# Immortalqx/pi-slam-fusion

Hardware: AMD Instinct MI355X
Metric: keyframes/sec fused (4000x3000 -> 256^2 tiles, 5-band) (higher is better)
Workload: dtype f32; 1 GPU; cfg-2/cfg-A: 4000x3000 BGR8 keyframes, serpentine sortie, Map2D.Scale=1, 5-band Laplacian, CV_32FC3 (ForceFloat=1) pyramids, frames resident in HBM; frames_per_rank=2646, sortie_frames_before_timing=20, lookahead=48, rendered_rank0=2666, culled_tiles_rank0=490117

## Files before the change

### include/pifusion.h

```cpp
#ifndef PIFUSION_H
#define PIFUSION_H
#include <stddef.h>
#include <stdint.h>

#ifdef __cplusplus
extern "C" {
#endif

#define PF_ELE_PIXELS 256

enum { PF_TYPE_NONE = 0, PF_TYPE_CPU = 1, PF_TYPE_GPU = 2, PF_TYPE_MULTIBAND = 3, PF_TYPE_RENDER = 4 };

enum { PF_8UC1 = 0, PF_8UC3 = 16, PF_8UC4 = 24, PF_16SC3 = 19, PF_32FC1 = 5, PF_32FC3 = 21 };

typedef struct pf_image {
    int         rows, cols, type;
    const void* data;
    size_t      step;
} pf_image;

typedef struct pf_options {
    int    band_number;
    int    force_float;
    int    high_quality_show;
// ... 126 lines not shown
int      pf_dist_blend_changed(pf_dist* d, int* xy, uint8_t* bgr, int cap);
int      pf_dist_save(pf_dist* d, const char* filename);
int      pf_dist_save_to_memory(pf_dist* d, uint8_t* bgr, int* rows, int* cols, int* tile_x0, int* tile_y0);
typedef struct pf_dist_stats {
    unsigned long long bytes_sent, bytes_received;
    unsigned long long strips_sent, strips_received, tiles, peers;
    double plan_ms, pack_ms, exchange_ms, compute_ms;
    unsigned long long verified;
} pf_dist_stats;
int      pf_dist_last_stats(pf_dist* d, pf_dist_stats* out);
typedef struct pf_strip_plan { int peer, ix, iy, dx, dy, tile; unsigned long long offset; } pf_strip_plan;
int      pf_dist_plan_blend(int nranks, int me, const int* counts, const int* lists3, const long long* caps, int high_quality,
                            const size_t halo_bytes9[9], pf_strip_plan* send, int send_cap, int* n_send,
                            pf_strip_plan* recv, int recv_cap, int* n_recv, int* mine_xy, int mine_cap, int* n_mine);
int      pf_dist_info(pf_dist* d, int* rank, int* nranks, const char** transport);
int      pf_dist_set_verify(pf_dist* d, int on);

int     pf_profile_enable(pf_map* m, int mode);
int     pf_profile_read(pf_map* m, int cap, const char** names, double* total_ms, long long* launches,
                        double* alg_bytes);
int     pf_profile_read_run(pf_map* m, int cap, const char** names, double* total_ms, long long* launches,
                            double* alg_bytes, double* alg_bytes_run);
int     pf_profile_reset(pf_map* m);
int     pf_render_stats(pf_map* m, double out4[4]);
int     pf_timer_read(pf_map* m, int cap, const char** names, long long* calls, double* mean_s, double* min_s, double* max_s);
int     pf_timer_reset(pf_map* m);
long long pf_debug_culled_tiles(pf_map* m);
long long pf_debug_culled_cells(pf_map* m);
double  pf_debug_level0_exact_px(pf_map* m);
int     pf_debug_render_log(pf_map* m, long long* out, int cap);
void    pf_set_cull(pf_map* m, int on);
void    pf_debug_form_counts(long long out[8]);
long long pf_debug_compact_launches(void);
int     pf_stats(pf_map* m, long long* rendered, long long* rejected, long long* dropped);
int     pf_reserve_tiles(pf_map* m, long long n_tiles);

#ifdef __cplusplus
}
#endif
#endif
```

### pi-slam-fusion_amd/__init__.py

```python
import ctypes as C
import os
import subprocess

import numpy as np

_HERE = os.path.dirname(os.path.abspath(__file__))
LIB_PATH = os.environ.get("PF_LIB") or os.path.join(_HERE, "libpifusion.so")
ELE_PIXELS = 256

NoType, TypeCPU, TypeGPU, TypeMultiBandCPU, TypeRender = 0, 1, 2, 3, 4
PF_8UC3, PF_8UC4, PF_16SC3, PF_32FC3 = 16, 24, 19, 21


def host_array(shape, dtype=np.uint8):
    n = int(np.prod(shape)) * np.dtype(dtype).itemsize
    p = lib().pf_host_alloc(n)
    if not p:
        raise MemoryError("pf_host_alloc(%d)" % n)
    buf = (C.c_uint8 * n).from_address(p)
    a = np.frombuffer(buf, dtype=dtype).reshape(shape)
    import weakref
    weakref.finalize(buf, lib().pf_host_free, p)
    return a

# ... 113 lines not shown
        L.pf_host_free.argtypes = [vp]; L.pf_host_free.restype = None
    if hasattr(L, "pf_blend_tiles_level") or not os.environ.get("PF_LIB"):
        L.pf_blend_tiles_level.argtypes = [vp, ip, C.c_int, C.c_int, vp, vp]
        L.pf_blend_changed_level.argtypes = [vp, C.c_int, ip, vp, C.c_int]
        L.pf_save_to_memory_level.argtypes = [vp, C.c_int, vp, ip, ip, ip, ip]
    L.pf_format_map_update.argtypes = [dp, dp, C.c_double, C.c_double, C.c_double, C.c_int, C.c_int, C.c_char_p, C.c_int]
    L.pf_map_update_command.argtypes = [vp, C.c_int, C.c_int, dp, C.c_char_p, C.c_int]
    L.pf_lnglat_from_distance.argtypes = [C.c_double, C.c_double, C.c_double, C.c_double, dp, dp]; L.pf_lnglat_from_distance.restype = None
    L.pf_normalize_using_weight_map.argtypes = [vp, vp, C.c_size_t]
    L.pf_mul_weight_map.argtypes = [vp, vp, C.c_size_t]
    L.pf_tile_owner.argtypes = [C.POINTER(Options), C.c_int, C.c_int]
    L.pf_halo_bytes.argtypes = [vp, C.c_int, C.c_int]; L.pf_halo_bytes.restype = C.c_size_t
    L.pf_halo_pack.argtypes = [vp, C.c_int, C.c_int, C.c_int, C.c_int, vp]
    L.pf_blend_tile_halo.argtypes = [vp, C.c_int, C.c_int, C.POINTER(vp), vp, vp]
    L.pf_tile_bytes.argtypes = [vp]; L.pf_tile_bytes.restype = C.c_size_t
    L.pf_tile_export.argtypes = [vp, C.c_int, C.c_int, vp]
    L.pf_tile_import.argtypes = [vp, C.c_int, C.c_int, vp]
    L.pf_dist_unique_id.argtypes = [vp]
    L.pf_dist_init_rccl.argtypes = [vp, vp, C.c_int, C.c_int]; L.pf_dist_init_rccl.restype = vp
    L.pf_dist_init_host.argtypes = [vp, C.c_int, C.c_int, EXCHANGE_FN, vp]; L.pf_dist_init_host.restype = vp
    L.pf_dist_destroy.argtypes = [vp]; L.pf_dist_destroy.restype = None
    L.pf_dist_blend_changed.argtypes = [vp, ip, vp, C.c_int]
    L.pf_dist_feed.argtypes = [vp, C.POINTER(Image), dp, C.c_int]
    L.pf_dist_feed_jpeg.argtypes = [vp, C.c_char_p, C.c_size_t, C.c_int, C.c_int, dp, C.c_int]
    L.pf_dist_save.argtypes = [vp, C.c_char_p]
    L.pf_dist_save_to_memory.argtypes = [vp, vp, ip, ip, ip, ip]
    L.pf_dist_last_stats.argtypes = [vp, C.POINTER(DistStats)]
    L.pf_dist_info.argtypes = [vp, ip, ip, C.POINTER(C.c_char_p)]
    L.pf_dist_set_verify.argtypes = [vp, C.c_int]
    L.pf_dist_plan_blend.argtypes = [C.c_int, C.c_int, ip, ip, C.POINTER(C.c_longlong), C.c_int, C.POINTER(C.c_size_t), vp, C.c_int, ip,
                                     vp, C.c_int, ip, ip, C.c_int, ip]
    if hasattr(L, "pf_debug_compact_launches") or not os.environ.get("PF_LIB"):
        L.pf_debug_compact_launches.argtypes = []; L.pf_debug_compact_launches.restype = C.c_longlong
    L.pf_profile_enable.argtypes = [vp, C.c_int]
    L.pf_profile_read.argtypes = [vp, C.c_int, C.POINTER(C.c_char_p), dp, C.POINTER(C.c_longlong), dp]
    if hasattr(L, "pf_profile_read_run") or not os.environ.get("PF_LIB"):
        L.pf_profile_read_run.argtypes = [vp, C.c_int, C.POINTER(C.c_char_p), dp, C.POINTER(C.c_longlong), dp, dp]
    L.pf_profile_reset.argtypes = [vp]
    L.pf_stats.argtypes = [vp, C.POINTER(C.c_longlong), C.POINTER(C.c_longlong), C.POINTER(C.c_longlong)]
    L.pf_reserve_tiles.argtypes = [vp, C.c_longlong]
    L.pf_debug_culled_tiles.argtypes = [vp]; L.pf_debug_culled_tiles.restype = C.c_longlong
    L.pf_set_cull.argtypes = [vp, C.c_int]; L.pf_set_cull.restype = None
    if hasattr(L, "pf_debug_render_log") or not os.environ.get("PF_LIB"):
        L.pf_debug_render_log.argtypes = [vp, C.POINTER(C.c_longlong), C.c_int]
    L.pf_debug_culled_cells.argtypes = [vp]; L.pf_debug_culled_cells.restype = C.c_longlong
    L.pf_debug_level0_exact_px.argtypes = [vp]; L.pf_debug_level0_exact_px.restype = C.c_double
    L.pf_render_stats.argtypes = [vp, dp]
    L.pf_timer_read.argtypes = [vp, C.c_int, C.POINTER(C.c_char_p), C.POINTER(C.c_longlong), dp, dp, dp]
    L.pf_timer_reset.argtypes = [vp]
    _lib = L
    return L


POSE7 = C.c_double * 7


def _pose(p):
    if isinstance(p, POSE7):
        return p, p
    a = np.ascontiguousarray(p, dtype=np.float64).reshape(-1)
    return a, a.ctypes.data_as(C.POINTER(C.c_double))


def default_options(**kw):
    o = Options()
    lib().pf_default_options(C.byref(o))
# ... 558 lines not shown
```

### pi-slam-fusion_amd/csrc/c_api.cpp

```cpp
#include "dist.hpp"
#include "jpeg_device.hpp"
#include "webtiles_plan.hpp"
#include <cerrno>
#include <map>
#include <string>
#include <sys/stat.h>
#include <cstdlib>
#include <cmath>
#include <cstdio>
#include <cstring>
#include <algorithm>
#include <vector>
#include <mutex>
#include <new>

using pf::FusionMap;

struct pf_map {
    FusionMap impl;
    pf::JpegDevice jpeg;
    pf_map(int t, bool th, const pf_options& o) : impl(t, th, o) {}
    ~pf_map() { if (impl.ok() && impl.use_device()) impl.sync(); }
};

// ... 27 lines not shown
    else if (!std::strcmp(key, "Map2D.Resolution")) o->resolution = v;
    else if (!std::strcmp(key, "Map2D.Scale")) o->scale = v;
    else if (!std::strcmp(key, "Device")) o->device = (int)v;
    else if (!std::strcmp(key, "Shard.Rank")) o->shard_rank = (int)v;
    else if (!std::strcmp(key, "Shard.Count")) o->shard_count = (int)v;
    else if (!std::strcmp(key, "Shard.Block")) o->shard_block = (int)v;
    else if (!std::strcmp(key, "Map2D.MaxQueue")) o->max_queue = (int)v;
    else if (!std::strcmp(key, "Fused")) o->fused = (int)v;
    else if (!std::strcmp(key, "Lookahead")) o->lookahead = (int)v;
    else return 0;
    return 1;
}

pf_map* pf_create(int type, int thread, const pf_options* opt)
{
    if (type == PF_TYPE_NONE || type == PF_TYPE_RENDER) return nullptr;
    pf_options o;
    if (opt) o = *opt; else pf_default_options(&o);
    pf_map* m = new (std::nothrow) pf_map(type, thread != 0, o);
    if (m && !m->impl.ok()) { delete m; return nullptr; }
    return m;
}

void pf_destroy(pf_map* m) { delete m; }
const char* pf_last_error(void) { return pf::last_error(); }

int pf_prepare(pf_map* m, const double plane[7], const double cam[6], int n, const pf_image* imgs, const double* poses7)
{ return m && m->impl.prepare(plane, cam, n, imgs, poses7); }

int pf_feed(pf_map* m, const pf_image* img, const double pose[7]) { return m && m->impl.feed(img, pose, false); }
int pf_feed_device(pf_map* m, const pf_image* img, const double pose[7]) { return m && m->impl.feed(img, pose, true); }
int pf_debug_phase_stamps(unsigned long long* out, int cap_blocks) { return pf::read_phase_stamps(out, cap_blocks); }
void pf_debug_form_counts(long long out[8]) { if (out) pf::read_form_counts(out); }
long long pf_debug_compact_launches(void) { return pf::read_compact_launches(); }
int pf_debug_render_log(pf_map* m, long long* out, int cap) { return m ? m->impl.render_log(out, cap) : 0; }
void pf_set_cull(pf_map* m, int on) { if (m) m->impl.set_cull(on != 0); }
long long pf_debug_culled_cells(pf_map* m) { return m ? m->impl.culled_cells() : 0; }
double pf_debug_level0_exact_px(pf_map* m) { return m ? m->impl.level0_exact_px() : 0; }
long long pf_debug_culled_tiles(pf_map* m) { return m ? m->impl.culled_tiles() : 0; }
int pf_debug_select_counts(unsigned long long* out, int reset) { return out ? pf::read_select_counts(out, reset) : 0; }
long pf_debug_read_last_frame(pf_map* m, void* out, size_t cap) { return m ? m->impl.read_back_last_frame(out, cap) : -1; }
unsigned pf_queue_size(pf_map* m) { return m ? m->impl.queue_size() : 0; }
int pf_sync(pf_map* m) { return m && m->impl.sync(); }
int pf_save(pf_map* m, const char* filename) { return m && filename && m->impl.save(filename); }
int pf_save_tiff(pf_map* m, const char* filename, int quality, int force_bigtiff) { return m && filename && m->impl.save_tiff(filename, quality, force_bigtiff != 0); }
int pf_save_tiff_masked(pf_map* m, const char* filename, int quality, int force_bigtiff) { return m && filename && m->impl.save_tiff_masked(filename, quality, force_bigtiff != 0); }
int pf_jpeg_info(const uint8_t* data, size_t len, int* rows, int* cols, int* components) { return pf::jpeg_info(data, len, rows, cols, components); }
int pf_jpeg_decode_bgr(const uint8_t* data, size_t len, uint8_t* bgr, int rows, int cols)
{ return rows > 0 && cols > 0 && pf::jpeg_decode_bgr(data, len, bgr, rows, cols, (size_t)cols * 3); }
int pf_jpeg_decode_device(const uint8_t* data, size_t len, void* dev_bgr, int rows, int cols, void* hip_stream)
{
    std::lock_guard<std::mutex> l(g_jpeg_mu);
    if (rows <= 0 || cols <= 0 || !dev_bgr) return 0;
    hipPointerAttribute_t at{};
    if (hipPointerGetAttributes(&at, dev_bgr) != hipSuccess || at.type != hipMemoryTypeDevice) { (void)hipGetLastError(); pf::set_error("pf_jpeg_decode_device: destination is not device memory"); return 0; }
    int prev = 0;
    (void)hipGetDevice(&prev);
    if (at.device != prev && hipSetDevice(at.device) != hipSuccess) { pf::set_error("pf_jpeg_decode_device: hipSetDevice failed"); return 0; }
    const int ok = shared_jpeg(at.device)->decode_to(data, len, (uint8_t*)dev_bgr, rows, cols, hip_stream);
    if (at.device != prev) (void)hipSetDevice(prev);
    return ok;
}
static pf::JpegEncoder* shared_jpeg_encoder(int device)
{
    static pf::JpegEncoder* e[64] = {};
    if (device < 0 || device >= 64) device = 0;
// ... 449 lines not shown
```

### pi-slam-fusion_amd/csrc/kernels.hip

```cpp
#include "kernels.hpp"
#include "warp_index.hpp"
#include "env.hpp"
#include <climits>
#include <cmath>
#include <cstdlib>
#include <type_traits>

#ifndef PF_EXPERIMENTS
#define PF_EXPERIMENTS 0
#endif
#ifndef PF_ROWTAB
#define PF_ROWTAB 0
#endif
#ifndef PF_HYBRID_W
#define PF_HYBRID_W 0
#endif

namespace pf {

constexpr bool kExp = PF_EXPERIMENTS != 0;

__device__ __forceinline__ double clamp_int_range(double v)
{
    v = (v < (double)INT_MAX) ? v : (double)INT_MAX;
    v = ((double)INT_MIN < v) ? v : (double)INT_MIN;
    return v;
}

#define PF_GLOBAL __attribute__((address_space(1)))
#ifdef PF_NT_STORES
#define PF_STORE(p, v) __builtin_nontemporal_store((v), (p))
#else
#define PF_STORE(p, v) (*(p) = (v))
#endif
#ifdef PF_NT_W
#define PF_STORE_W(p, v) __builtin_nontemporal_store((v), (p))
#define PF_LOAD_W(p) __builtin_nontemporal_load(p)
#else
#define PF_STORE_W(p, v) (*(p) = (v))
#define PF_LOAD_W(p) (*(p))
#endif
#ifdef PF_NT_SRC
// ... 221 lines not shown
                       int ty0, int ty1, int tx0, int tx1)
{
    const int ts = kElePixels >> level;
    const int px0 = tx0 * ts, px1 = tx1 * ts, py0 = ty0 * ts, py1 = ty1 * ts;
    if (px1 <= px0 || py1 <= py0) return;
    dim3 grid((px1 - px0 + 63) / 64, (py1 - py0 + 3) / 4), block(256);
    if (lay.f32) hipLaunchKernelGGL(k_lap_select<true>, grid, block, 0, s, lay, level, g_i, g_up, w_i, rows, cols, tile_table, tiles_x, py0, px0, px1, py1);
    else         hipLaunchKernelGGL(k_lap_select<false>, grid, block, 0, s, lay, level, g_i, g_up, w_i, rows, cols, tile_table, tiles_x, py0, px0, px1, py1);
}

typedef float f2 __attribute__((ext_vector_type(2)));
typedef float f4 __attribute__((ext_vector_type(4)));
template <bool F32> struct PxT;
template <> struct alignas(16) PxT<true>  { float c[3]; float w; };
template <> struct alignas(4)  PxT<false> { short c[3]; short pad; float w; };
template <bool F32> struct alignas(16) HxT { typename Pix<F32>::WT c[3]; float w; };

typedef unsigned short us2 __attribute__((ext_vector_type(2)));
typedef short ss2 __attribute__((ext_vector_type(2)));
struct __attribute__((may_alias)) alignas(4) PxP { us2 c01, c2p; float w; };
struct __attribute__((may_alias)) alignas(4) BxP { ss2 c01, c2p; };

constexpr int LBW = 64, LAW = LBW + 7, LQW = LBW / 2 + 2;

struct LevelOffsets { uint32_t lap_off, w_off, top_lap_off, top_w_off; };
struct FusedWarp {
    double M[9];
    long   total;
    const float* wmap;
    int    srows, scols, sstep, cn;
    int    plain;
    float  wxc, wyc, wdmax, wrcp;
    int    wtype;
    int    seed_ok;
    float  Mf[9];
    int    phx, phy;
    int    pitch_i, pitch_w;
};

struct LevelArgs {
    int level, rows, cols;
    int cx0, cy0, cx1, cy1;
    int tiles_x;
    int top_select;
    int write_next;
    int nbx, nby;
    int ablate;
    int seg;
    unsigned inv_nbx;
    int pad_;
};
template <class GA>
__device__ __forceinline__ void block_xy(const GA& g, int b, int& bx, int& by)
{
    if (g.inv_nbx) by = (int)__umulhi((unsigned)b, g.inv_nbx); else by = b / g.nbx;
    bx = b - by * g.nbx;
}

__device__ __forceinline__ double rcp_mid_range(double d)
{
    double r = __builtin_amdgcn_rcp(d);
    double e = __builtin_fma(-d, r, 1.0); r = __builtin_fma(r, e, r);
    e = __builtin_fma(-d, r, 1.0); r = __builtin_fma(r, e, r);
    const double rem = __builtin_fma(-d, r, 1.0);
    return __builtin_fma(rem, r, r);
}
// ... 683 lines not shown
                        if (hasb) Aat(rb, c) = pb;
                    } else {
                        Aat(r, c) = warp_pixel<F32>(src, wa, col, y);
                        if (hasb) Aat(rb, c) = warp_pixel<F32>(src, wa, col, yb);
                    }
                }
            }
        } else
        if (ILP == 0 && WA && inner && wa.plain && block_maps_inside(wa, ax0, ay0, LAW, LAH)) {
            constexpr bool kRowTab = PF_ROWTAB != 0;
            double (*rowtab)[3][4] = reinterpret_cast<double (*)[3][4]>(tail);
            const int xb0 = ax0 & ~63;
            if constexpr (kRowTab) {
                static_assert(!kRowTab || sizeof(double) * LAH * 3 * 4 <= (size_t)kTail, "row table fits behind A");
                if (tid < LAH * 9) {
                    const int r = tid / 9, e = tid - r * 9, kx = e / 3, w = e - kx * 3;
                    const double xb = (double)(xb0 + 64 * kx), y = (double)(ay0 + r);
                    rowtab[r][kx][w] = wa.M[3 * w] * xb + wa.M[3 * w + 1] * y + wa.M[3 * w + 2];
                }
                lds_barrier();
            }
            if (r0 < RS) {
                constexpr int NR = (LAH + RS - 1) / RS;
                typedef uint32_t u2 __attribute__((ext_vector_type(2), aligned(1)));
                using p2 = typename std::conditional<F32, park8, park4>::type;
                const WarpCol col = warp_col(wa, ax0 + c);
                const int cn = wa.cn, sstep = wa.sstep;
                constexpr int CH = (F32 && LBH != 24) ? NR : (NR + 1) / 2;
                u2 b0[CH], b1[CH];
                float wq[(CH + 1) / 2] = {};
                const int rbase = r0 * NR;
                const bool seed = kExp && wa.seed_ok != 0;
                double Wn = 0.0;
#pragma unroll
                for (int h = 0; h < NR; h += CH) {
#pragma unroll
                    for (int k = h; k < h + CH && k < NR; k++) {
                        const bool has = rbase + k < LAH;
                        if (k >= LAH - (RS - 1) * NR && __builtin_amdgcn_ballot_w64(has) == 0) continue;
                        const int r = has ? rbase + k : rbase;
                        const int y = ay0 + r;
                        double X0, Y0, W0;
                        if constexpr (kRowTab) {
                            const double* t = rowtab[r][(((ax0 + c) & ~63) - xb0) >> 6];
                            X0 = t[0]; Y0 = t[1]; W0 = t[2];
                        } else {
                            X0 = col.m0xb + wa.M[1] * y + wa.M[2]; Y0 = col.m3xb + wa.M[4] * y + wa.M[5]; W0 = col.m6xb + wa.M[7] * y + wa.M[8];
                        }
                        const double W = W0 + col.m6x1, xn = X0 + col.m0x1, yn = Y0 + col.m3x1;
                        Wn = (k > 0 && seed) ? rcp_seeded(W, Wn) : rcp_mid_range(W);
                        const double pxn = xn * Wn, pyn = yn * Wn;
                        constexpr double kMagic = 6755399441055744.0;
                        const int Xn = (int)(uint32_t)(unsigned long long)__double_as_longlong(pxn + kMagic);
                        const int Yn = (int)(uint32_t)(unsigned long long)__double_as_longlong(pyn + kMagic);
                        const int X = (int)(uint32_t)(unsigned long long)__double_as_longlong(__builtin_fma(pxn, 32., kMagic));
                        const int Y = (int)(uint32_t)(unsigned long long)__double_as_longlong(__builtin_fma(pyn, 32., kMagic));
                        constexpr bool kHyb = PF_HYBRID_W != 0; const bool gw_row = kHyb && (k & 1);
                        float wgt;
                        if (gw_row) wgt = *(const float*)((const char*)wa.wmap + ((uint32_t)(__mul24(Yn, wa.scols) + Xn) << 2));
                        else wgt = radial_weight(wa, Xn, Yn);
                        const uint32_t off0 = (uint32_t)(__mul24(Y >> 5, sstep) + __mul24(cn, X >> 5));
                        if (gw_row) wq[(k - h) >> 1] = wgt;
                        if (has) *reinterpret_cast<p2*>(&Aat(r, c)) = p2{ (uint32_t)((X & 31) | (Y & 31) << 5), __float_as_uint(gw_row ? 0.f : wgt) };
                        b0[k - h] = PF_LOAD_SRC((const u2*)(src + off0)); b1[k - h] = PF_LOAD_SRC((const u2*)(src + off0 + (uint32_t)sstep));
                    }
#pragma unroll
                    for (int k = h; k < h + CH && k < NR; k++) {
                        const bool has = rbase + k < LAH;
                        if (k >= LAH - (RS - 1) * NR && __builtin_amdgcn_ballot_w64(has) == 0) continue;
                        if (!has) continue;
                        const int r = rbase + k;
                        const p2 pk = *reinterpret_cast<const p2*>(&Aat(r, c));
                        constexpr bool kHyb = PF_HYBRID_W != 0; const bool gw_row = kHyb && (k & 1);
                        Aat(r, c) = warp_finish_fast<F32>(b0[k - h].x, b0[k - h].y, b1[k - h].x, b1[k - h].y, (int)(pk.x & 31u), (int)(pk.x >> 5), gw_row ? wq[(k - h) >> 1] : __uint_as_float(pk.y), cn);
                    }
                }
            }
        } else
        if (r0 < RS) {
            const int x = col_of(c);
            const WarpCol col = warp_col(wa, x);
            if constexpr (ILP == 3) {
                for (int r = r0; r < LAH; r += 3 * RS) {
                    const int rb = r + RS, rc = r + 2 * RS;
                    const bool hasb = rb < LAH, hasc = rc < LAH;
                    const int y = row_of(r), yb = row_of(hasb ? rb : r), yc = row_of(hasc ? rc : r);
                    if (kExp && (g.ablate & 1)) { Px z{}; z.w = (float)(x + y); Aat(r, c) = z; if (hasb) Aat(rb, c) = z; if (hasc) Aat(rc, c) = z; continue; }
                    const WarpTaps ta = warp_fetch<WA>(src, wa, col, y);
                    const WarpTaps tb = warp_fetch<WA>(src, wa, col, yb);
                    if (__builtin_amdgcn_ballot_w64(hasc) != 0) {
                        const WarpTaps tc = warp_fetch<WA>(src, wa, col, yc);
                        Aat(r, c) = warp_finish<F32>(ta, wa.cn);
                        if (hasb) Aat(rb, c) = warp_finish<F32>(tb, wa.cn);
                        if (hasc) Aat(rc, c) = warp_finish<F32>(tc, wa.cn);
                    } else {
                        Aat(r, c) = warp_finish<F32>(ta, wa.cn);
                        if (hasb) Aat(rb, c) = warp_finish<F32>(tb, wa.cn);
// ... 503 lines not shown
    const int pitch_i = (15 + (pw - 2) * cn + 8 + 15) & ~15, pitch_w = (15 + pw * 4 + 15) & ~15;
    if ((pitch_i >> 4) + (pitch_w >> 4) > 64) return false;
    if ((long)ph * (pitch_i + pitch_w) > kPatchBytes) return false;
    for (int i = 0; i < 9; i++) w.Mf[i] = (float)M[i];
    w.phx = hx; w.phy = hy; w.pitch_i = pitch_i; w.pitch_w = pitch_w;
    return true;
}

#endif

static unsigned level_inv_nbx(int nbx, int nby)
{
    if (nbx <= 1 || (unsigned long long)nbx * nby * nbx >= 0x100000000ull) return 0;
    return (unsigned)((0x100000000ull + (unsigned)nbx - 1) / (unsigned)nbx);
}

static int seed_plan(const double* M, int rows, int cols)
{
    static const bool on = kExp && getenv("PF_SEED") != nullptr;
    if (!on) return 0;
    const double xs[2] = { -4.0, cols + 3.0 }, ys[2] = { -4.0, rows + 3.0 };
    double wmin = 0; int sign = 0;
    for (int i = 0; i < 4; i++) {
        const double W = M[6] * xs[i & 1] + M[7] * ys[i >> 1] + M[8];
        if (!(std::fabs(W) > 0x1p-400) || !std::isfinite(W)) return 0;
        const int sg = W > 0 ? 1 : -1;
        if (sign && sg != sign) return 0;
        sign = sg;
        wmin = i ? std::min(wmin, std::fabs(W)) : std::fabs(W);
    }
    return std::fabs(M[7]) <= 0x1p-16 * wmin;
}

size_t level_px_bytes(bool f32) { return f32 ? sizeof(PxT<true>) : sizeof(PxT<false>); }

void launch_level(hipStream_t s, const TileLayout& lay, int level, int rows, int cols, int cx0, int cy0, int cx1, int cy1,
                  int tiles_x, bool top_select, bool write_next, const WarpArgs* wa, const uint8_t* src,
                  const void* gw_in, void* gw_out, const uint64_t* table, int shape)
{
    LevelArgs g{};
    g.level = level; g.rows = rows; g.cols = cols; g.cx0 = cx0; g.cy0 = cy0; g.cx1 = cx1; g.cy1 = cy1;
    g.tiles_x = tiles_x; g.top_select = top_select; g.write_next = write_next;
    static const int force = exp_env_int("PF_KLEVEL", 0);
    static const int ablate = kExp && getenv("PF_ABLATE") ? atoi(getenv("PF_ABLATE")) : 0;
    const bool use4 = force == 4 || (force != 3 && shape == 2);
    const int BH = use4 ? 16 : 32;
    const int LSTEPS = 1;
    g.nbx = (cx1 - cx0 + LBW - 1) / LBW; g.nby = (cy1 - cy0 + BH * LSTEPS - 1) / (BH * LSTEPS);
    g.inv_nbx = level_inv_nbx(g.nbx, g.nby);
    g.ablate = ablate;
    if (g.nbx <= 0 || g.nby <= 0) return;
    dim3 grid(g.nbx * g.nby);
    FusedWarp w{};
    if (wa) {
        for (int i = 0; i < 9; i++) w.M[i] = wa->M[i];
        w.total = frame_bytes(wa->srows, wa->scols, wa->sstep, wa->src_cn); w.wmap = wa->wmap;
        w.srows = wa->srows; w.scols = wa->scols; w.sstep = (int)wa->sstep; w.cn = wa->src_cn;
        w.plain = plain_homography(*wa);
    }
    LevelOffsets lo{ lay.lap_off[level], lay.w_off[level], lay.lap_off[level + 1], lay.w_off[level + 1] };
#define PF_LAUNCH(K, F, W, ...) hipLaunchKernelGGL((K<F, W, __VA_ARGS__>), grid, dim3(512), 0, s, lo, g, w, src, (const PxT<F>*)gw_in, (PxT<F>*)gw_out, table)
    if (use4) {
        if (lay.f32) { if (wa) PF_LAUNCH(k_level, true, true, 16, 512, 1); else PF_LAUNCH(k_level, true, false, 16, 512, 1); }
        else         { if (wa) PF_LAUNCH(k_level, false, true, 16, 512, 1); else PF_LAUNCH(k_level, false, false, 16, 512, 1); }
    } else {
        if (lay.f32) { if (wa) PF_LAUNCH(k_level3, true, true, 32, 512); else PF_LAUNCH(k_level3, true, false, 32, 512); }
        else         { if (wa) PF_LAUNCH(k_level3, false, true, 32, 512); else PF_LAUNCH(k_level3, false, false, 32, 512); }
    }
#undef PF_LAUNCH
}


static unsigned long long* g_stamp_buf = nullptr;
static int g_stamp_blocks = 0;
[[maybe_unused]] constexpr int kStampBlocks = 1 << 16;

static long long g_form_counts[8] = {};
void read_form_counts(long long out[8]) { for (int i = 0; i < 8; i++) out[i] = g_form_counts[i]; }
static long long g_compact_launches = 0;
long long read_compact_launches() { return g_compact_launches; }

#if PF_EXPERIMENTS
static bool launch_strips(hipStream_t s, const TileLayout& lay, const LevelLaunch* jobs, int njobs, const WarpArgs* wa, const uint8_t* src)
{
    static const int on = getenv("PF_STRIPS") ? atoi(getenv("PF_STRIPS")) : 0;
    static const int sablate = getenv("PF_SABLATE") ? atoi(getenv("PF_SABLATE")) : 0;
    static const bool stamp = getenv("PF_STAMP") != nullptr;
    static const bool other = getenv("PF_WEIGHT_PLANE") || getenv("PF_PATCH") || getenv("PF_BLOCK64") || getenv("PF_ABLATE") || getenv("PF_A_ILP");
    static const int order = getenv("PF_UPPER_FIRST") ? 2 : (getenv("PF_INTERLEAVE_JOBS") ? 0 : 1);
    if (!on || other) return false;
    if (wa && !radial_weight_exact(*wa)) return false;
    constexpr int R = 4;
    static const int seg_env = getenv("PF_STRIP_SEG") ? atoi(getenv("PF_STRIP_SEG")) : 0;
    const int seg = seg_env >= R ? (seg_env / R) * R : 64;
    LevelBatch batch{};
    int first_blocks = 0, upper_blocks = 0;
    for (int k = 0; k < njobs; k++) {
        const LevelLaunch& q = jobs[k];
        LevelJob& J = batch.job[batch.njobs];
        J.g.level = q.level; J.g.rows = q.rows; J.g.cols = q.cols; J.g.cx0 = q.cx0; J.g.cy0 = q.cy0; J.g.cx1 = q.cx1; J.g.cy1 = q.cy1;
        J.g.tiles_x = q.tiles_x; J.g.top_select = q.top_select; J.g.write_next = q.write_next; J.g.ablate = sablate;
        J.g.seg = seg;
        J.g.nbx = (q.cx1 - q.cx0 + strips::KW - 1) / strips::KW; J.g.nby = (q.cy1 - q.cy0 + seg - 1) / seg;
        if (J.g.nbx <= 0 || J.g.nby <= 0) continue;
        if ((q.cx0 | q.cy0 | q.cy1) & 1) return false;
        J.lay = LevelOffsets{ lay.lap_off[q.level], lay.w_off[q.level], lay.lap_off[q.level + 1], lay.w_off[q.level + 1] };
        J.gw_in = q.gw_in; J.gw_out = q.gw_out; J.table = q.table; J.from_warp = q.from_warp;
        {
            const int cap = batch.njobs == 0 ? kMaxRects : kMaxRectsUpper;
            J.nrect = q.nrect;
            if (q.nrect > cap) {
// ... 116 lines not shown
        if (ok && total > 0 && total * 4 <= (long)J0.g.nbx * J0.g.nby * 3 && total < (1l << 24)) {
            batch.compact0 = (int)total;
            first_blocks = (int)((total + 7) & ~7l);
            g_compact_launches++;
        }
    }
    const int nblocks = first_blocks + upper_blocks;
    batch.upper_groups = upper_blocks / 8; batch.total_groups = nblocks / 8;
    batch.sequential = 1;
    if (kExp) {
        static const bool interleave = getenv("PF_INTERLEAVE_JOBS") != nullptr;
        static const bool upper_first = getenv("PF_UPPER_FIRST") != nullptr;
        batch.sequential = upper_first ? 2 : !interleave;
        static const int rect_runs = getenv("PF_RECT_ORDER") ? atoi(getenv("PF_RECT_ORDER")) : 0;
        batch.rect_runs = rect_runs;
    }
    if (batch.njobs && batch.job[0].from_warp && batch.job[0].g.level == 0) batch.need_r0 = level0_need_reach(lay, batch.tab0_n, batch.job[0].nrect);
#if PF_EXPERIMENTS
    static const bool force_test = getenv("PF_FORCE_NEED_TEST") != nullptr;
    if (force_test && batch.njobs && batch.job[0].from_warp && batch.job[0].g.level == 0 && batch.tab0_n > 0 && batch.job[0].nrect == 0 && !batch.need_r0) {
        batch.need_r0 = level0_need_reach(lay, batch.tab0_n, 1);
        if (batch.need_r0) { batch.job[0].nrect = 1; batch.rect0[0] = BlockRect{ 0, 0, 32767, 32767 }; }
    }
#endif
    if (!batch.njobs) return;
    FusedWarp w{};
    if (wa) {
        for (int i = 0; i < 9; i++) w.M[i] = wa->M[i];
        w.total = frame_bytes(wa->srows, wa->scols, wa->sstep, wa->src_cn); w.wmap = wa->wmap;
        w.srows = wa->srows; w.scols = wa->scols; w.sstep = (int)wa->sstep; w.cn = wa->src_cn;
        w.plain = plain_homography(*wa);
        w.wxc = wa->xc; w.wyc = wa->yc; w.wdmax = wa->dis_max; w.wrcp = (float)(1.0L / (long double)wa->dis_max); w.wtype = wa->weight_type;
        w.seed_ok = (w.plain && batch.job[0].from_warp) ? seed_plan(wa->M, batch.job[0].g.rows, batch.job[0].g.cols) : 0;
    }
    if (batch.tab0_n) g_form_counts[7]++;
    static const bool wplane_env = exp_env("PF_WEIGHT_PLANE") != nullptr;
    const bool wplane = wplane_env || (wa && !radial_weight_exact(*wa));
    unsigned long long* st = nullptr;
#if PF_EXPERIMENTS
    static const bool stamp = getenv("PF_STAMP") != nullptr;
    static const int ilp_env = getenv("PF_A_ILP") ? atoi(getenv("PF_A_ILP")) : -1;
    if (stamp && BH == 32) {
        if (!g_stamp_buf) { if (hipMalloc((void**)&g_stamp_buf, kStampBlocks * 64) != hipSuccess) g_stamp_buf = nullptr; }
        if (g_stamp_buf && nblocks <= kStampBlocks) {
            (void)hipMemsetAsync(g_stamp_buf, 0, (size_t)kStampBlocks * 64, s);
            g_stamp_blocks = nblocks;
            st = g_stamp_buf;
        }
    }
#define PF_GO(F, H, T, S, I, P, W) hipLaunchKernelGGL((k_levels<F, H, T, S, I, P, W>), dim3(nblocks), dim3(T), 0, s, batch, w, src, st)
    if (st) {
        g_form_counts[6]++;
        if (wplane) { if (lay.f32) PF_GO(true, 32, 512, true, 3, false, false); else PF_GO(false, 32, 512, true, 2, false, false); }
        else        { if (lay.f32) PF_GO(true, 32, 512, true, 0, false, true);  else PF_GO(false, 32, 512, true, 2, false, true); }
        return;
    }
    if (wa && batch.job[0].from_warp && patch_plan(*wa, batch.job[0].g.rows, batch.job[0].g.cols, BH, w)) {
        g_form_counts[2]++;
        if (lay.f32) PF_GO(true, 32, 512, false, 2, true, false); else PF_GO(false, 32, 512, false, 2, true, false);
        return;
    }
    if (BH == 24) {
        if (wa) g_form_counts[5]++;
        if (lay.f32) PF_GO(true, 24, 512, false, 0, false, true); else PF_GO(false, 24, 512, false, 2, false, true);
        return;
    }
    if (BH == 28) {
        if (wa) g_form_counts[5]++;
        if (wplane) { if (lay.f32) PF_GO(true, 28, 512, false, 3, false, false); else PF_GO(false, 28, 512, false, 2, false, false); }
        else        { if (lay.f32) PF_GO(true, 28, 512, false, 3, false, true);  else PF_GO(false, 28, 512, false, 2, false, true); }
        return;
    }
    if (BH == 64) {
        if (wa) g_form_counts[4]++;
        if (lay.f32) PF_GO(true, 64, 1024, false, 3, false, false); else PF_GO(false, 64, 1024, false, 2, false, false);
        return;
    }
    if (ilp_env == 0 && !wplane && !lay.f32) {
        if (wa) g_form_counts[0]++;
        PF_GO(false, 32, 512, false, 0, false, true);
        return;
    }
    if (ilp_env == 2 || ilp_env == 3) {
        if (wa) g_form_counts[wplane ? 1 : 0]++;
        if (wplane) {
            if (lay.f32) { if (ilp_env == 3) PF_GO(true, 32, 512, false, 3, false, false); else PF_GO(true, 32, 512, false, 2, false, false); }
            else         { if (ilp_env == 3) PF_GO(false, 32, 512, false, 3, false, false); else PF_GO(false, 32, 512, false, 2, false, false); }
        } else {
            if (lay.f32) { if (ilp_env == 3) PF_GO(true, 32, 512, false, 3, false, true); else PF_GO(true, 32, 512, false, 2, false, true); }
            else         { if (ilp_env == 3) PF_GO(false, 32, 512, false, 3, false, true); else PF_GO(false, 32, 512, false, 2, false, true); }
        }
        return;
    }
#undef PF_GO
#endif
    if (wa) g_form_counts[wplane ? 1 : 0]++;
    if (wplane) {
        if (lay.f32) hipLaunchKernelGGL((k_levels<true, 32, 512, false, 3, false, false>), dim3(nblocks), dim3(512), 0, s, batch, w, src, st);
        else         hipLaunchKernelGGL((k_levels<false, 32, 512, false, 2, false, false>), dim3(nblocks), dim3(512), 0, s, batch, w, src, st);
    } else {
        if (lay.f32) hipLaunchKernelGGL((k_levels<true, 32, 512, false, 0, false, true>), dim3(nblocks), dim3(512), 0, s, batch, w, src, st);
        else         hipLaunchKernelGGL((k_levels<false, 32, 512, false, 2, false, true>), dim3(nblocks), dim3(512), 0, s, batch, w, src, st);
    }
}

int level_block_rows(bool f32)
{
    (void)f32;
#if PF_EXPERIMENTS
    static const bool b64 = getenv("PF_BLOCK64") != nullptr, b28 = getenv("PF_BLOCK28") != nullptr, b24 = getenv("PF_BLOCK24") != nullptr;
    return b64 ? 64 : (b28 ? 28 : (b24 ? 24 : 32));
#else
    return 32;
#endif
}

int read_select_counts(unsigned long long* out, int reset)
{
    unsigned long long seen[kMaxLevels], won[kMaxLevels];
    if (hipMemcpyFromSymbol(seen, HIP_SYMBOL(g_select_seen), sizeof seen) != hipSuccess) return 0;
    if (hipMemcpyFromSymbol(won, HIP_SYMBOL(g_select_won), sizeof won) != hipSuccess) return 0;
    for (int i = 0; i < kMaxLevels; i++) { out[2 * i] = seen[i]; out[2 * i + 1] = won[i]; }
    if (reset) {
        unsigned long long z[kMaxLevels] = {};
        (void)hipMemcpyToSymbol(HIP_SYMBOL(g_select_seen), z, sizeof z); (void)hipMemcpyToSymbol(HIP_SYMBOL(g_select_won), z, sizeof z);
    }
    return kMaxLevels;
}

// ... 248 lines not shown
```

### pi-slam-fusion_amd/csrc/kernels.hpp

```cpp
#pragma once
#include "plan_limits.hpp"
#include <hip/hip_runtime.h>
#include <cstdint>
#include <cstddef>

namespace pf {

struct TileLayout {
    int      nlev;
    int      f32;
    uint32_t lap_off[kMaxLevels];
    uint32_t w_off[kMaxLevels];
    uint32_t slot_bytes;
};

TileLayout make_layout(int band_num, bool f32);

struct WarpArgs {
    double M[9];
    int    srows, scols;
    long   sstep;
    int    crows, ccols;
    int    y_off, x_off;
    int    wrows, wcols;
// ... 19 lines not shown

enum KernelId { K_WARP = 0, K_PYRDOWN_IMG, K_PYRDOWN_W, K_LAP_SELECT, K_BLEND_GATHER, K_COLLAPSE,
                K_BLEND_FINISH, K_MOSAIC_GATHER, K_SAVE_FINISH, K_LEVEL0, K_LEVEL, K_SINGLE, K_BLEND_FUSED, K_SAVE_FUSED, K_BLEND_LEVEL, K_SAVE_LEVEL, K_COUNT };
const char* kernel_name(int id);

void launch_warp(hipStream_t s, bool f32, const uint8_t* src, const WarpArgs& a, void* g0, float* w0);

void launch_pyrdown(hipStream_t s, int type, const void* src, int srows, int scols, void* dst,
                    int y0, int y1, int x0, int x1);

void launch_lap_select(hipStream_t s, const TileLayout& lay, int level, const void* g_i, const void* g_up,
                       const float* w_i, int rows, int cols, const uint64_t* tile_table, int tiles_x,
                       int ty0, int ty1, int tx0, int tx1);

size_t level_px_bytes(bool f32);
void launch_level(hipStream_t s, const TileLayout& lay, int level, int rows, int cols, int cx0, int cy0, int cx1, int cy1,
                  int tiles_x, bool top_select, bool write_next, const WarpArgs* wa, const uint8_t* src,
                  const void* gw_in, void* gw_out, const uint64_t* table, int shape = 3);

struct LevelLaunch {
    int level, rows, cols;
    int cx0, cy0, cx1, cy1;
    int tiles_x;
    bool top_select, write_next, from_warp;
    const void* gw_in; void* gw_out;
    const uint64_t* table;
    const uint64_t* table_args; int table_n;
    int nrect; BlockRect rect[kMaxRects];
    const uint32_t* need_bits = nullptr; int need_n = 0;
};
void launch_levels(hipStream_t s, const TileLayout& lay, const LevelLaunch* jobs, int njobs, const WarpArgs* wa, const uint8_t* src);
int  read_phase_stamps(unsigned long long* out, int cap_blocks);
void read_form_counts(long long out[8]);
long long read_compact_launches();
int  read_select_counts(unsigned long long* out, int reset);
int  level0_need_reach(const TileLayout& lay, int table_n, int nrect0);
int  level_block_rows(bool f32);

void launch_blend_fused(hipStream_t s, const TileLayout& lay, const BlendJob* jobs_dev, int n, void* raw_out, uint8_t* bgr_out);
void launch_save_fused(hipStream_t s, const TileLayout& lay, const uint64_t* table_dev, int wx, int wy, int bg, uint8_t* bgr_out);
void launch_blend_level(hipStream_t s, const TileLayout& lay, int level, const BlendJob* jobs_dev, int n, void* raw_out, uint8_t* bgr_out);
void launch_save_level(hipStream_t s, const TileLayout& lay, int level, const uint64_t* table_dev, int wx, int wy, int bg, uint8_t* bgr_out);

void launch_blend_gather(hipStream_t s, const TileLayout& lay, int level, int border, const BlendSrc* srcs,
                         void* dst, size_t dst_stride_bytes, int batch);
void launch_collapse(hipStream_t s, bool f32, void* dst, size_t dst_stride_bytes, const void* src,
                     size_t src_stride_bytes, int rows, int cols, int batch);
void launch_blend_finish(hipStream_t s, const TileLayout& lay, const void* lvl0, size_t stride_bytes, int border,
                         const BlendSrc* srcs, void* raw_out, uint8_t* bgr_out, int batch, const int* out_idx = nullptr);

void launch_mosaic_gather(hipStream_t s, const TileLayout& lay, int level, const uint64_t* table, int wx, int wy, void* dst);
void launch_save_finish(hipStream_t s, const TileLayout& lay, const void* lvl0, const uint64_t* table, int wx, int wy,
                        int bg, uint8_t* bgr);

size_t halo_bytes(const TileLayout& lay, int dx, int dy);
void launch_halo_pack(hipStream_t s, const TileLayout& lay, const void* slot, int dx, int dy, void* out);
struct StripDesc { const void* slot; int dx, dy; size_t out_off; };
void launch_halo_pack_batch(hipStream_t s, const TileLayout& lay, const StripDesc* descs_dev, int n, void* out);

void launch_weight8(hipStream_t s, uint8_t* w, int rows, int cols, int weight_type);
void launch_weight32(hipStream_t s, float* w, int rows, int cols, int weight_type);
void launch_single(hipStream_t s, const uint8_t* src, const uint8_t* w8, const WarpArgs& a, const uint64_t* table, int tiles_x);

}
```

Before: 26200 keyframes/s.

## Add incremental float delta stepping for homography warp coordinates with proven error bound

Adds a level-0 warp path that computes one exact double-precision anchor row per thread. Neighbouring rows' source coordinates are then stepped with cheap float Taylor-style deltas. A host-side planner derives an error bound `eps`, and any pixel near a rounding boundary falls back to the exact double chain, chosen by wave ballot. The goal is to cut the per-pixel double-precision divide and projection cost in the warp/pyramid kernel, at the price of extra code complexity, register pressure and divergence on fallback. It is gated behind the `PF_DELTA_PATH` compile flag, which defaults to `PF_EXPERIMENTS`, and a `PF_DELTA` environment toggle. A debug launch counter is also added.

```diff
diff --git a/include/pifusion.h b/include/pifusion.h
--- a/include/pifusion.h
+++ b/include/pifusion.h
@@ -182,6 +182,7 @@
 void    pf_set_cull(pf_map* m, int on);
 void    pf_debug_form_counts(long long out[8]);
 long long pf_debug_compact_launches(void);
+long long pf_debug_delta_launches(void);
 int     pf_stats(pf_map* m, long long* rendered, long long* rejected, long long* dropped);
 int     pf_reserve_tiles(pf_map* m, long long n_tiles);
 
diff --git a/pi-slam-fusion_amd/__init__.py b/pi-slam-fusion_amd/__init__.py
--- a/pi-slam-fusion_amd/__init__.py
+++ b/pi-slam-fusion_amd/__init__.py
@@ -169,6 +169,8 @@
                                      vp, C.c_int, ip, ip, C.c_int, ip]
     if hasattr(L, "pf_debug_compact_launches") or not os.environ.get("PF_LIB"):
         L.pf_debug_compact_launches.argtypes = []; L.pf_debug_compact_launches.restype = C.c_longlong
+    if hasattr(L, "pf_debug_delta_launches") or not os.environ.get("PF_LIB"):
+        L.pf_debug_delta_launches.argtypes = []; L.pf_debug_delta_launches.restype = C.c_longlong
     L.pf_profile_enable.argtypes = [vp, C.c_int]
     L.pf_profile_read.argtypes = [vp, C.c_int, C.POINTER(C.c_char_p), dp, C.POINTER(C.c_longlong), dp]
     if hasattr(L, "pf_profile_read_run") or not os.environ.get("PF_LIB"):
diff --git a/pi-slam-fusion_amd/csrc/c_api.cpp b/pi-slam-fusion_amd/csrc/c_api.cpp
--- a/pi-slam-fusion_amd/csrc/c_api.cpp
+++ b/pi-slam-fusion_amd/csrc/c_api.cpp
@@ -83,6 +83,7 @@
 int pf_feed_device(pf_map* m, const pf_image* img, const double pose[7]) { return m && m->impl.feed(img, pose, true); }
 int pf_debug_phase_stamps(unsigned long long* out, int cap_blocks) { return pf::read_phase_stamps(out, cap_blocks); }
 void pf_debug_form_counts(long long out[8]) { if (out) pf::read_form_counts(out); }
+long long pf_debug_delta_launches(void) { return pf::read_delta_launches(); }
 long long pf_debug_compact_launches(void) { return pf::read_compact_launches(); }
 int pf_debug_render_log(pf_map* m, long long* out, int cap) { return m ? m->impl.render_log(out, cap) : 0; }
 void pf_set_cull(pf_map* m, int on) { if (m) m->impl.set_cull(on != 0); }
diff --git a/pi-slam-fusion_amd/csrc/kernels.hip b/pi-slam-fusion_amd/csrc/kernels.hip
--- a/pi-slam-fusion_amd/csrc/kernels.hip
+++ b/pi-slam-fusion_amd/csrc/kernels.hip
@@ -1,13 +1,18 @@
 #include "kernels.hpp"
 #include "warp_index.hpp"
+#include "warp_delta.hpp"
 #include "env.hpp"
 #include <climits>
+#include <cstdio>
 #include <cmath>
 #include <cstdlib>
 #include <type_traits>
 
 #ifndef PF_EXPERIMENTS
 #define PF_EXPERIMENTS 0
+#endif
+#ifndef PF_DELTA_PATH
+#define PF_DELTA_PATH PF_EXPERIMENTS
 #endif
 #ifndef PF_ROWTAB
 #define PF_ROWTAB 0
@@ -295,6 +300,7 @@
     int    plain;
     float  wxc, wyc, wdmax, wrcp;
     int    wtype;
+    float  delta_eps;
     int    seed_ok;
     float  Mf[9];
     int    phx, phy;
@@ -1044,8 +1050,54 @@
                 const int rbase = r0 * NR;
                 const bool seed = kExp && wa.seed_ok != 0;
                 double Wn = 0.0;
+                constexpr bool kDelta = PF_DELTA_PATH != 0 && F32 && ILP == 0 && WA && LBH == 32 && LNT == 512 && CH == NR && NR == kDeltaRows && !kRowTab && PF_HYBRID_W == 0;
+                static_assert(!kDelta || (RS - 1) * NR + kDeltaAnchor < LAH, "every thread has its anchor row");
+                const float deps = kDelta ? wa.delta_eps : 0.f;
+                if (kDelta && deps > 0.f) {
+                    constexpr double kMagic = 6755399441055744.0;
+                    const int x = ax0 + c;
+                    auto chain = [&](int y, double& pxn, double& pyn, double& Wr, int& X, int& Y, int& Xn, int& Yn) {
+                        const WarpCol cl = warp_col(wa, x);
+                        const double X0 = cl.m0xb + wa.M[1] * y + wa.M[2], Y0 = cl.m3xb + wa.M[4] * y + wa.M[5], W0 = cl.m6xb + wa.M[7] * y + wa.M[8];
+                        const double W = W0 + cl.m6x1, xn = X0 + cl.m0x1, yn = Y0 + cl.m3x1;
+                        Wr = rcp_mid_range(W);
+                        pxn = xn * Wr; pyn = yn * Wr;
+                        Xn = (int)(uint32_t)(unsigned long long)__double_as_longlong(pxn + kMagic);
+                        Yn = (int)(uint32_t)(unsigned long long)__double_as_longlong(pyn + kMagic);
+                        X = (int)(uint32_t)(unsigned long long)__double_as_longlong(__builtin_fma(pxn, 32., kMagic));
+                        Y = (int)(uint32_t)(unsigned long long)__double_as_longlong(__builtin_fma(pyn, 32., kMagic));
+                    };
+                    auto emit = [&](int k, bool has, int X, int Y, int Xn, int Yn) {
+                        const float wgt = radial_weight(wa, Xn, Yn);
+                        const uint32_t off0 = (uint32_t)(__mul24(Y >> 5, sstep) + __mul24(cn, X >> 5));
+                        if (has) *reinterpret_cast<p2*>(&Aat(rbase + k, c)) = p2{ (uint32_t)((X & 31) | (Y & 31) << 5), __float_as_uint(wgt) };
+                        b0[k] = PF_LOAD_SRC((const u2*)(src + off0)); b1[k] = PF_LOAD_SRC((const u2*)(src + off0 + (uint32_t)sstep));
+                    };
+                    DeltaAnchor an;
+                    {
+                        double pxn, pyn, Wr; int X, Y, Xn, Yn;
+                        chain(ay0 + rbase + kDeltaAnchor, pxn, pyn, Wr, X, Y, Xn, Yn);
+                        an = delta_anchor(wa.M[1], wa.M[4], wa.M[7], pxn, pyn, Wr, X, Y);
+                        emit(kDeltaAnchor, true, X, Y, Xn, Yn);
+                    }
+                    auto row = [&](auto kc) {
+                        constexpr int k = decltype(kc)::value;
+                        const bool has = rbase + k < LAH;
+                        if (k >= LAH - (RS - 1) * NR && __builtin_amdgcn_ballot_w64(has) == 0) return;
+                        DeltaPx q = delta_step<k - kDeltaAnchor>(an, deps);
+                        if (!has) { q.X = an.X; q.Y = an.Y; q.ok = true; }
+                        if (__builtin_expect(__builtin_amdgcn_ballot_w64(!q.ok) != 0, 0)) {
+                            double pxn, pyn, Wr;
+                            chain(ay0 + (has ? rbase + k : rbase), pxn, pyn, Wr, q.X, q.Y, q.Xn, q.Yn);
+                        }
+                        emit(k, has, q.X, q.Y, q.Xn, q.Yn);
+                    };
+                    row(std::integral_constant<int, 0>{}); row(std::integral_constant<int, 1>{}); row(std::integral_constant<int, 3>{});
+                    row(std::integral_constant<int, 4>{}); row(std::integral_constant<int, 5>{});
+                }
 #pragma unroll
                 for (int h = 0; h < NR; h += CH) {
+                    if (!(kDelta && deps > 0.f)) {
 #pragma unroll
                     for (int k = h; k < h + CH && k < NR; k++) {
                         const bool has = rbase + k < LAH;
@@ -1075,6 +1127,7 @@
                         if (gw_row) wq[(k - h) >> 1] = wgt;
                         if (has) *reinterpret_cast<p2*>(&Aat(r, c)) = p2{ (uint32_t)((X & 31) | (Y & 31) << 5), __float_as_uint(gw_row ? 0.f : wgt) };
                         b0[k - h] = PF_LOAD_SRC((const u2*)(src + off0)); b1[k - h] = PF_LOAD_SRC((const u2*)(src + off0 + (uint32_t)sstep));
+                    }
                     }
 #pragma unroll
                     for (int k = h; k < h + CH && k < NR; k++) {
@@ -1644,6 +1697,23 @@
     return std::fabs(M[7]) <= 0x1p-16 * wmin;
 }
 
+static float delta_eps_for(const double* M, int rows, int cols, int srows, int scols, int plain)
+{
+    static const bool off = exp_env_int("PF_DELTA", 1) == 0;
+    static const double raised = exp_env_double("PF_DELTA_EPS", 0.0);
+    if (off) return 0.f;
+    const float eps = delta_plan(M, rows, cols, srows, scols, plain);
+    if (eps > 0.f && raised != 0.0) {
+        if (!(raised >= (double)eps)) {
+            static bool told = false;
+            if (!told) { told = true; fprintf(stderr, "pifusion: PF_DELTA_EPS=%g is below the planned bound %g: refused, the planned bound holds\n", raised, (double)eps); }
+            return eps;
+        }
+        return (float)raised;
+    }
+    return eps;
+}
+
 size_t level_px_bytes(bool f32) { return f32 ? sizeof(PxT<true>) : sizeof(PxT<false>); }
 
 void launch_level(hipStream_t s, const TileLayout& lay, int level, int rows, int cols, int cx0, int cy0, int cx1, int cy1,
@@ -1689,6 +1759,8 @@
 
 static long long g_form_counts[8] = {};
 void read_form_counts(long long out[8]) { for (int i = 0; i < 8; i++) out[i] = g_form_counts[i]; }
+static long long g_delta_launches = 0;
+long long read_delta_launches() { return g_delta_launches; }
 static long long g_compact_launches = 0;
 long long read_compact_launches() { return g_compact_launches; }
 
@@ -1871,10 +1943,13 @@
         w.plain = plain_homography(*wa);
         w.wxc = wa->xc; w.wyc = wa->yc; w.wdmax = wa->dis_max; w.wrcp = (float)(1.0L / (long double)wa->dis_max); w.wtype = wa->weight_type;
         w.seed_ok = (w.plain && batch.job[0].from_warp) ? seed_plan(wa->M, batch.job[0].g.rows, batch.job[0].g.cols) : 0;
+        if (PF_DELTA_PATH != 0 && lay.f32 && batch.job[0].from_warp && batch.job[0].g.level == 0 && radial_weight_exact(*wa))
+            w.delta_eps = delta_eps_for(wa->M, batch.job[0].g.rows, batch.job[0].g.cols, wa->srows, wa->scols, w.plain);
     }
     if (batch.tab0_n) g_form_counts[7]++;
     static const bool wplane_env = exp_env("PF_WEIGHT_PLANE") != nullptr;
     const bool wplane = wplane_env || (wa && !radial_weight_exact(*wa));
+    if (wplane) w.delta_eps = 0.f;
     unsigned long long* st = nullptr;
 #if PF_EXPERIMENTS
     static const bool stamp = getenv("PF_STAMP") != nullptr;
@@ -1892,6 +1967,7 @@
         g_form_counts[6]++;
         if (wplane) { if (lay.f32) PF_GO(true, 32, 512, true, 3, false, false); else PF_GO(false, 32, 512, true, 2, false, false); }
         else        { if (lay.f32) PF_GO(true, 32, 512, true, 0, false, true);  else PF_GO(false, 32, 512, true, 2, false, true); }
+        if (!wplane && lay.f32 && w.delta_eps > 0.f) g_delta_launches++;
         return;
     }
     if (wa && batch.job[0].from_warp && patch_plan(*wa, batch.job[0].g.rows, batch.job[0].g.cols, BH, w)) {
@@ -1934,6 +2010,7 @@
 #undef PF_GO
 #endif
     if (wa) g_form_counts[wplane ? 1 : 0]++;
+    if (!wplane && lay.f32 && w.delta_eps > 0.f) g_delta_launches++;
     if (wplane) {
         if (lay.f32) hipLaunchKernelGGL((k_levels<true, 32, 512, false, 3, false, false>), dim3(nblocks), dim3(512), 0, s, batch, w, src, st);
         else         hipLaunchKernelGGL((k_levels<false, 32, 512, false, 2, false, false>), dim3(nblocks), dim3(512), 0, s, batch, w, src, st);
diff --git a/pi-slam-fusion_amd/csrc/kernels.hpp b/pi-slam-fusion_amd/csrc/kernels.hpp
--- a/pi-slam-fusion_amd/csrc/kernels.hpp
+++ b/pi-slam-fusion_amd/csrc/kernels.hpp
@@ -75,6 +75,7 @@
 void launch_levels(hipStream_t s, const TileLayout& lay, const LevelLaunch* jobs, int njobs, const WarpArgs* wa, const uint8_t* src);
 int  read_phase_stamps(unsigned long long* out, int cap_blocks);
 void read_form_counts(long long out[8]);
+long long read_delta_launches();
 long long read_compact_launches();
 int  read_select_counts(unsigned long long* out, int reset);
 int  level0_need_reach(const TileLayout& lay, int table_n, int nrect0);
diff --git a/pi-slam-fusion_amd/csrc/warp_delta.hpp b/pi-slam-fusion_amd/csrc/warp_delta.hpp
--- /dev/null
+++ b/pi-slam-fusion_amd/csrc/warp_delta.hpp
@@ -0,0 +1,109 @@
+#pragma once
+#include <cmath>
+#include <cstdint>
+
+#if defined(__HIPCC__)
+#define PF_WD_HD __host__ __device__ __forceinline__
+#else
+#define PF_WD_HD inline
+#endif
+
+namespace pf {
+
+constexpr int kDeltaRows = 6, kDeltaAnchor = 2, kDeltaKMax = 3;
+
+struct DeltaAnchor {
+    float t, ax, ay;
+    float fx, fy;
+    int   X, Y;
+};
+
+#if defined(__HIP_DEVICE_COMPILE__)
+PF_WD_HD double wd_fma(double a, double b, double c) { return __builtin_fma(a, b, c); }
+PF_WD_HD float  wd_fmaf(float a, float b, float c) { return __builtin_fmaf(a, b, c); }
+PF_WD_HD float  wd_rint(float v) { return __builtin_rintf(v); }
+PF_WD_HD float  wd_abs(float v) { return __builtin_fabsf(v); }
+#else
+PF_WD_HD double wd_fma(double a, double b, double c) { return std::fma(a, b, c); }
+PF_WD_HD float  wd_fmaf(float a, float b, float c) { return std::fmaf(a, b, c); }
+PF_WD_HD float  wd_rint(float v) { return std::nearbyintf(v); }
+PF_WD_HD float  wd_abs(float v) { return std::fabs(v); }
+#endif
+
+PF_WD_HD DeltaAnchor delta_anchor(double M1, double M4, double M7, double pxn, double pyn, double Wn, int X, int Y)
+{
+    DeltaAnchor a;
+    const double w32 = 32. * Wn;
+    a.t  = (float)(M7 * Wn);
+    a.ax = (float)(wd_fma(-pxn, M7, M1) * w32);
+    a.ay = (float)(wd_fma(-pyn, M7, M4) * w32);
+    a.fx = (float)wd_fma(pxn, 32., -(double)X);
+    a.fy = (float)wd_fma(pyn, 32., -(double)Y);
+    a.X = X; a.Y = Y;
+    return a;
+}
+
+struct DeltaPx { int X, Y, Xn, Yn; bool ok; float dx, dy; };
+
+PF_WD_HD bool delta_coord(float f, float ka, float u, int X0, float lim, int& X, int& Xn, float& d)
+{
+    const float s = wd_fmaf(ka, u, f);
+    const float r = wd_rint(s);
+    d = s - r;
+    X = X0 + (int)r;
+    Xn = (X + 15 + (d > 0.f ? 1 : 0)) >> 5;
+    return wd_abs(wd_abs(d) - 0.25f) < lim;
+}
+
+template <int K>
+PF_WD_HD DeltaPx delta_step(const DeltaAnchor& a, float eps)
+{
+    const float kt = (float)K * a.t;
+    const float u = (1.f - kt) + kt * kt;
+    const float lim = 0.25f - eps;
+    DeltaPx o;
+    const bool okx = delta_coord(a.fx, (float)K * a.ax, u, a.X, lim, o.X, o.Xn, o.dx);
+    const bool oky = delta_coord(a.fy, (float)K * a.ay, u, a.Y, lim, o.Y, o.Yn, o.dy);
+    o.ok = okx && oky;
+    return o;
+}
+
+inline float delta_plan(const double* M, int crows, int ccols, int srows, int scols, int plain)
+{
+    if (!plain || crows <= 0 || ccols <= 0 || srows <= 0 || scols <= 0) return 0.f;
+    const double xs[2] = { -8.0, ccols + 8.0 }, ys[2] = { -8.0, crows + 8.0 };
+    double dmin = 0; int sign = 0;
+    for (int i = 0; i < 4; i++) {
+        const double D = M[6] * xs[i & 1] + M[7] * ys[i >> 1] + M[8];
+        if (!std::isfinite(D) || !(std::fabs(D) > 0x1p-400)) return 0.f;
+        const int sg = D > 0 ? 1 : -1;
+        if (sign && sg != sign) return 0.f;
+        sign = sg;
+        dmin = i ? std::fmin(dmin, std::fabs(D)) : std::fabs(D);
+    }
+    const double u24 = 0x1p-24, u53 = 0x1p-53, K = kDeltaKMax;
+    const double wn = (1.0 / dmin) * (1 + 0x1p-50);
+    const double xmax = ccols + 72.0, ymax = crows + 8.0;
+    const double nabs = std::fmax(std::fabs(M[0]) * xmax + std::fabs(M[1]) * ymax + std::fabs(M[2]),
+                                  std::fabs(M[3]) * xmax + std::fabs(M[4]) * ymax + std::fabs(M[5]));
+    const double dabs = std::fabs(M[6]) * xmax + std::fabs(M[7]) * ymax + std::fabs(M[8]);
+    const double pmax = srows > scols ? srows : scols;
+    const double tau = K * std::fabs(M[7]) * wn;
+    if (!(tau <= 0x1p-10)) return 0.f;
+    const double amax = 32. * wn * std::fmax(std::fabs(M[1]) + scols * std::fabs(M[7]), std::fabs(M[4]) + srows * std::fabs(M[7]));
+    const double alpha = K * amax;
+    const double e_ref = 32. * u53 * (6. * nabs * wn + pmax * (6. * dabs * wn + 2.));
+    const double eta = u53 * (6. * dabs * wn + 3.);
+    const double dt = u24 + eta;
+    const double dA = amax * (u24 + 2. * u53 + eta) + tau / K * e_ref;
+    const double eu = 2. * u24 + u24 * tau * tau + (1. + 2. * tau) * tau * (dt + u24) + tau * tau * tau / (1. - tau);
+    const double es = alpha * eu + (1. + 2. * tau) * (K * dA + u24 * alpha) + u24 * alpha * (1. + 2. * tau)
+                    + u24 * (0.5 + alpha * (1. + 2. * tau)) + 0x1p-26;
+    const double proven = (2. * e_ref + es) * (1. + 0x1p-10);
+    const double eps = 2. * proven;
+    if (!std::isfinite(eps) || !(eps <= 0x1p-10)) return 0.f;
+    const float ef = (float)eps;
+    return (double)ef >= eps ? ef : std::nextafterf(ef, 1.f);
+}
+
+}
```

Result: slower. 23690 keyframes/s (-9.6%).
